# m4tx/idencomp

Measured on NVIDIA B200. Metric: fastq_compress_decompress_GBps, higher is better.
Workload: dtype u32

## Files before the change

idencomp_b200/csrc/idn_device.cuh:

```cuda
#pragma once
#include <cstdint>
#include <cuda_runtime.h>

namespace idn {

constexpr uint32_t kScaleBits = 14;
constexpr uint32_t kAcidSyms = 5, kQSyms = 94;
constexpr uint32_t kSlotMask = (1u << kScaleBits) - 1;
constexpr uint32_t kRansL = 1u << 23;
constexpr int kHist = 8;
constexpr int kQLutBytes = 128;
#ifndef IDN_QROW352
constexpr int kQWindows = 24;
constexpr int kQRowBytes = kQLutBytes + 16 * kQWindows;
#else
constexpr int kQStarts = 104;
constexpr int kQRowBytes = 352;
#endif
constexpr int kQWinBytes = 128 * 16;

struct Magic {
    uint32_t m, s;
};
__host__ __device__ constexpr Magic make_magic(uint32_t d) {
// ... 24 lines not shown
    uint32_t pb;
    uint32_t sbits;
    uint32_t asub, qmul, light;
};

struct SpecBuild {
    SpecDev spec;
    uint32_t total_bits;
    bool ok;
};

__host__ __device__ constexpr uint64_t spec_ipow(uint64_t b, uint32_t n) {
    uint64_t r = 1;
    while (n--) r *= b;
    return r;
}
__host__ __device__ constexpr uint32_t spec_bitlen(uint64_t v) {
    uint32_t n = 0;
    while (v) {
        n++;
        v >>= 1;
    }
    return n;
}

__host__ __device__ constexpr bool make_queue(uint32_t base, uint32_t order, QueueDev& q, uint32_t& bits) {
    q = QueueDev{0, 0, 0, 0, 0, 0, 0, 0, order};
    uint64_t pw = spec_ipow(base, order);
    if (pw > (1ull << 31)) return false;
    bits = spec_bitlen(pw - 1);
    if (order == 0) return true;
    q.vmul = 1;
    uint32_t M = (uint32_t)spec_ipow(base, order - 1);
    q.powmul = M;
    Magic mb = make_magic(base);
    q.mb = mb.m;
    q.shb = mb.s;
    if (order >= 2) {
        q.B = base;
        Magic mm = make_magic(M);
        q.m = mm.m;
        q.sh = mm.s;
        q.MB = (uint32_t)((uint64_t)M * base);
    }
    return true;
}

__host__ __device__ constexpr SpecBuild make_spec(int kind, int ao, int qo, int pb, int qmax) {
    SpecBuild r{SpecDev{QueueDev{0, 0, 0, 0, 0, 0, 0, 0, 0}, QueueDev{0, 0, 0, 0, 0, 0, 0, 0, 0}, 0, 0, 0, 0, 0, 0}, 0, false};
    if (kind != 0 && kind != 1) return r;
    if (ao < 0 || ao > kHist || qo < 0 || qo > kHist || pb < 0 || pb > 16) return r;
    SpecDev& s = r.spec;
    s.pb = (uint32_t)pb;
    s.light = kind == 1;
    uint32_t base_a = 5, base_q = 94;
    s.asub = 0;
    s.qmul = 1u << 20;
    if (s.light) {
        if (qmax < 1 || qmax > 94) return r;
        base_a = 4;
        base_q = (uint32_t)qmax;
        s.asub = 1;
        s.qmul = (uint32_t)qmax * 11156u;
        for (uint32_t q = 0; q < 94; q++)
            if (((q * s.qmul) >> 20) != q * (uint32_t)qmax / 94) return r;
    }
    uint32_t qbits = 0;
    if (!make_queue(base_a, (uint32_t)ao, s.qa, s.abits)) return r;
    if (base_q == 1) {
        s.qq = QueueDev{0, 0, 0, 0, 0, 0, 0, 0, (uint32_t)qo};
        qbits = 0;
    } else if (!make_queue(base_q, (uint32_t)qo, s.qq, qbits)) {
        return r;
    }
    if (s.abits + qbits + s.pb > 31) return r;
    s.sbits = s.abits + qbits;
    r.total_bits = s.abits + qbits + s.pb;
    r.ok = true;
    return r;
}

struct DynSpecs {
    static constexpr bool kStatic = false;
    static constexpr bool kQWin = false;
    __host__ __device__ static constexpr SpecDev sa() { return make_spec(0, 0, 0, 0, 0).spec; }
    __host__ __device__ static constexpr SpecDev sq() { return make_spec(0, 0, 0, 0, 0).spec; }
};
template <int KA, int AOA, int QOA, int PBA, int QMA, int KQ, int AOQ, int QOQ, int PBQ, int QMQ>
struct StaticSpecs {
    static constexpr bool kStatic = true;
#ifdef IDN_QWIN_ALL
    static constexpr bool kQWin = true;
#elif defined(IDN_QWIN_NONE)
    static constexpr bool kQWin = false;
#else
    static constexpr bool kQWin = KQ == 0 && AOQ == 2 && QOQ == 1 && PBQ == 6;
#endif
    __host__ __device__ static constexpr SpecDev sa() { return make_spec(KA, AOA, QOA, PBA, QMA).spec; }
    __host__ __device__ static constexpr SpecDev sq() { return make_spec(KQ, AOQ, QOQ, PBQ, QMQ).spec; }
};

struct ModelDev {
    SpecDev spec;
    uint32_t type, nsym, n_rows;
    const uint16_t* map;
    const uint32_t* hkeys;
    const uint32_t* hvals;
    uint32_t hmask;
    const uint2* enc;
    const uint8_t* dec;
    const uint4* qwin;
    const uint2* adirect;
    const uint2* aenc;
};

__device__ __forceinline__ uint2 ldg_stream8(const uint2* p) {
#ifdef IDN_ACID_NOALLOC
    uint2 v;
    asm volatile("ld.global.nc.L1::no_allocate.v2.u32 {%0, %1}, [%2];" : "=r"(v.x), "=r"(v.y) : "l"(p));
    return v;
#else
    return __ldg(p);
#endif
}

__device__ __forceinline__ uint32_t hash32(uint32_t k) {
    k ^= k >> 16;
    k *= 0x7feb352dU;
    k ^= k >> 15;
    k *= 0x846ca68bU;
    k ^= k >> 16;
    return k;
}

__host__ __device__ constexpr uint32_t spec_table_index(const SpecDev& s, uint32_t spec) {
    return s.pb == 0 ? spec : (((spec & ((1u << s.pb) - 1u)) << s.sbits) | (spec >> s.pb));
}

__device__ __forceinline__ uint32_t ctx_row_hash(const ModelDev& m, uint32_t spec) {
    if (!m.hkeys) return 0;
    uint32_t h = hash32(spec) & m.hmask;
    for (;;) {
        uint32_t k = __ldg(m.hkeys + h);
        if (k == spec) return __ldg(m.hvals + h);
        if (k == 0xffffffffu) return 0;
        h = (h + 1) & m.hmask;
    }
}

template <bool kDense = false, class Gen>
__device__ __forceinline__ uint32_t gen_row(const ModelDev& m, const SpecDev& s, const Gen& g, uint32_t pos_shared, uint32_t pshift) {
    if (kDense || m.map) return __ldg(m.map + g.index(s, pos_shared, pshift));
    return ctx_row_hash(m, g.spec(s, pos_shared, pshift));
}

__device__ __forceinline__ void map_syms(const SpecDev& s, uint32_t a, uint32_t q, bool z, uint32_t& va, uint32_t& vq) {
    va = a - s.asub;
    vq = (q * s.qmul) >> 20;
    const bool kill = z && s.light != 0;
    va = kill ? 0u : va;
    vq = kill ? 0u : vq;
}

__device__ __forceinline__ uint32_t queue_push(const QueueDev& k, uint32_t s, uint32_t v) {
    uint32_t q = __umulhi(s, k.m) >> k.sh;
    return s * k.B - q * k.MB + v * k.vmul;
}
__device__ __forceinline__ uint32_t queue_slide_back(const QueueDev& k, uint32_t s, uint32_t v_old) {
    return (__umulhi(s, k.mb) >> k.shb) + v_old * k.powmul;
}

struct PosFwd {
    uint32_t pos, rem, step, frac, len;
    __device__ __forceinline__ void init(uint32_t length, uint32_t pbmax) {
        len = length ? length : 1;
        uint32_t P = 1u << pbmax;
        step = P / len;
        frac = P - step * len;
        pos = rem = 0;
    }
    __device__ __forceinline__ void init_at(uint32_t length, uint32_t pbmax, uint32_t i) {
        init(length, pbmax);
        const unsigned long long t = (unsigned long long)i << pbmax;
        pos = (uint32_t)(t / len);
        rem = (uint32_t)(t % len);
    }
    __device__ __forceinline__ void advance() {
        pos += step;
        rem += frac;
        if (rem >= len) {
            rem -= len;
            pos++;
        }
    }
};
struct PosBack {
    uint32_t pos, rem, step, frac, len;
    __device__ __forceinline__ void init(uint32_t length, uint32_t pbmax) {
        len = length ? length : 1;
        uint32_t P = 1u << pbmax;
        step = P / len;
        frac = P - step * len;
        pos = P;
        rem = 0;
    }
    __device__ __forceinline__ void init_at(uint32_t length, uint32_t pbmax, uint32_t i) {
        init(length, pbmax);
        const unsigned long long t = (unsigned long long)i << pbmax;
        pos = (uint32_t)(t / len);
        rem = (uint32_t)(t % len);
    }
    __device__ __forceinline__ void retreat() {
        pos -= step;
        if (rem < frac) {
            rem += len;
            pos--;
        }
        rem -= frac;
    }
};

struct GenFwd {
    uint32_t sa, sq;
    __device__ __forceinline__ void init() { sa = sq = 0; }
    __device__ __forceinline__ uint32_t spec(const SpecDev& s, uint32_t pos_shared, uint32_t pshift) const {
        if (s.pb == 0) return (sq << s.abits) | sa;
        return (((sq << s.abits) | sa) << s.pb) | (pos_shared >> pshift);
    }
    __device__ __forceinline__ uint32_t index(const SpecDev& s, uint32_t pos_shared, uint32_t pshift) const {
        if (s.pb == 0) return (sq << s.abits) | sa;
        return ((pos_shared >> pshift) << s.sbits) | ((sq << s.abits) | sa);
    }
    __device__ __forceinline__ void update(const SpecDev& s, uint32_t a, uint32_t q, bool z) {
        uint32_t va, vq;
        map_syms(s, a, q, z, va, vq);
        sa = queue_push(s.qa, sa, va);
        sq = queue_push(s.qq, sq, vq);
    }
};

struct GenBack {
    uint32_t sa, sq;
    uint32_t wa;
    unsigned long long wq;
    uint32_t sha, shq;

    __device__ __forceinline__ void clear(const SpecDev& s) {
        sa = sq = 0;
        wa = 0;
        wq = 0;
        sha = 3 * s.qa.depth;
        shq = 7 * s.qq.depth;
    }
    __device__ __forceinline__ void shift_in(const SpecDev& s, uint32_t a, uint32_t q, bool z) {
        uint32_t va, vq;
        map_syms(s, a, q, z, va, vq);
        wa = (wa >> 3) | (va << (3 * kHist));
        wq = (wq >> 7) | ((unsigned long long)vq << (7 * kHist));
    }
    __device__ __forceinline__ void init_state(const SpecDev& s) {
        sa = sq = 0;
        for (uint32_t k = s.qa.depth; k >= 1; k--) sa = queue_push(s.qa, sa, (wa >> (3 * k)) & 7u);
        for (uint32_t k = s.qq.depth; k >= 1; k--) sq = queue_push(s.qq, sq, (uint32_t)(wq >> (7 * k)) & 127u);
    }
    __device__ __forceinline__ void step_back(const SpecDev& s) {
        sa = queue_slide_back(s.qa, sa, (wa >> sha) & 7u);
        sq = queue_slide_back(s.qq, sq, (uint32_t)(wq >> shq) & 127u);
    }
    __device__ __forceinline__ uint32_t spec(const SpecDev& s, uint32_t pos_shared, uint32_t pshift) const {
        if (s.pb == 0) return (sq << s.abits) | sa;
        return (((sq << s.abits) | sa) << s.pb) | (pos_shared >> pshift);
    }
    __device__ __forceinline__ uint32_t index(const SpecDev& s, uint32_t pos_shared, uint32_t pshift) const {
        if (s.pb == 0) return (sq << s.abits) | sa;
        return ((pos_shared >> pshift) << s.sbits) | ((sq << s.abits) | sa);
    }
};

template <class Out>
__device__ __forceinline__ void rans_put_bf(uint32_t& x, uint2 e, Out& out) {
    const uint32_t freq = (e.y >> 14) & 0x3fffu;
    const uint32_t start = e.y & 0x3fffu;
    const uint32_t x_max = freq << (23 - kScaleBits + 8);
    const bool one = x >= x_max, two = (x >> 8) >= x_max;
    const uint32_t sel = two ? 0x4401u : (one ? 0x4440u : 0x4444u);
    const uint32_t kbits = two ? 16u : (one ? 8u : 0u);
    out.push_bits(__byte_perm(x, 0, sel), kbits);
    x >>= kbits;
    const uint32_t q = freq == 1 ? x : (__umulhi(x, e.x) >> (e.y >> 28));
    x = x + start + q * ((1u << kScaleBits) - freq);
}

__device__ __forceinline__ void rans_put_count(uint32_t& x, uint2 e, uint32_t& bytes) {
    uint32_t freq = (e.y >> 14) & 0x3fffu;
    uint32_t start = e.y & 0x3fffu;
    uint32_t x_max = freq << (23 - kScaleBits + 8);
    const uint32_t k = (x >= x_max ? 1u : 0u) + ((x >> 8) >= x_max ? 1u : 0u);
    bytes += k;
    x >>= 8 * k;
    uint32_t q = freq == 1 ? x : (__umulhi(x, e.x) >> (e.y >> 28));
    x = x + start + q * ((1u << kScaleBits) - freq);
}

__device__ __forceinline__ uint32_t acid_find(uint2 packed, uint32_t slot, uint32_t& start, uint32_t& freq) {
    const uint32_t c1 = packed.x & 0xffffu, c2 = packed.x >> 16, c3 = packed.y & 0xffffu, c4 = packed.y >> 16;
    const bool p1 = slot >= c1, p2 = slot >= c2, p3 = slot >= c3, p4 = slot >= c4;
    start = p4 ? c4 : (p3 ? c3 : (p2 ? c2 : (p1 ? c1 : 0u)));
    const uint32_t next = !p1 ? c1 : (!p2 ? c2 : (!p3 ? c3 : (!p4 ? c4 : (1u << kScaleBits))));
    freq = next - start;
    return p4 ? 4u : (p3 ? 3u : (p2 ? 2u : (p1 ? 1u : 0u)));
}

#ifndef IDN_QROW352
__device__ __forceinline__ uint32_t q_find(const uint8_t* __restrict__ row, uint32_t slot, uint32_t& start,
                                           uint32_t& freq) {
    uint32_t g = __ldg(row + (slot >> 7));
    const uint4* wins = reinterpret_cast<const uint4*>(row + kQLutBytes);
    const uint32_t K = (slot | 0x8000u) * 0x10001u;
    uint4 w = __ldg(wins + g);
    uint32_t flags;
    for (;;) {
        flags = ((K - w.x) & 0x80008000u) | (((K - w.y) & 0x80008000u) >> 1) | (((K - w.z) & 0x80008000u) >> 2) |
                (((K - w.w) & 0x80008000u) >> 3);
#ifndef IDN_ABL_NOADV
        if (!(flags & 0x10000000u)) break;
        g++;
        w = __ldg(wins + g);
#else
        break;
#endif
    }
    const uint32_t j = __popc(flags) - 1;
    const uint32_t p = j >> 1;
    const uint32_t w0 = p == 0 ? w.x : (p == 1 ? w.y : (p == 2 ? w.z : w.w));
    const uint32_t w1 = p == 0 ? w.y : (p == 1 ? w.z : w.w);
    const uint32_t pair = __funnelshift_r(w0, w1, 16 * (j & 1));
    start = pair & 0xffffu;
    freq = (pair >> 16) - start;
    return 4 * g + j;
}
#else
__device__ __forceinline__ uint32_t q_find(const uint8_t* __restrict__ row, uint32_t slot, uint32_t& start,
                                           uint32_t& freq) {
    uint32_t g = __ldg(row + (slot >> 7));
    const uint2* starts = reinterpret_cast<const uint2*>(row + kQLutBytes);
    const uint32_t K = (slot | 0x8000u) * 0x10001u;
    uint2 lo = __ldg(starts + g), hi = __ldg(starts + g + 1);
    uint32_t flags;
    for (;;) {
        flags = ((K - lo.x) & 0x80008000u) | (((K - lo.y) & 0x80008000u) >> 1) | (((K - hi.x) & 0x80008000u) >> 2) |
                (((K - hi.y) & 0x80008000u) >> 3);
        if (!(flags & 0x10000000u)) break;
        g++;
        lo = hi;
        hi = __ldg(starts + g + 1);
    }
    const uint32_t j = __popc(flags) - 1;
    const uint32_t p = j >> 1;
    const uint32_t w0 = p == 0 ? lo.x : (p == 1 ? lo.y : (p == 2 ? hi.x : hi.y));
    const uint32_t w1 = p == 0 ? lo.y : (p == 1 ? hi.x : hi.y);
    const uint32_t pair = __funnelshift_r(w0, w1, 16 * (j & 1));
    start = pair & 0xffffu;
    freq = (pair >> 16) - start;
    return 4 * g + j;
}
#endif

__device__ __forceinline__ uint32_t q_find_win(const uint4* __restrict__ win_row, const uint8_t* __restrict__ row, uint32_t slot,
                                               uint32_t& start, uint32_t& freq) {
    const uint4 w = __ldg(win_row + (slot >> 7));
    const uint32_t K = (slot | 0x8000u) * 0x10001u;
    const uint32_t flags = ((K - w.y) & 0x80008000u) | (((K - w.z) & 0x80008000u) >> 1) | (((K - w.w) & 0x80008000u) >> 2);
    const uint32_t j = __popc(flags);
    if (j == 6) return q_find(row, slot, start, freq);
    const uint32_t i = j + 1;
    const uint32_t p = i >> 1;
    const uint32_t w0 = p == 0 ? w.x : (p == 1 ? w.y : (p == 2 ? w.z : w.w));
    const uint32_t w1 = p == 0 ? w.y : (p == 1 ? w.z : w.w);
    const uint32_t pair = __funnelshift_r(w0, w1, 16 * (i & 1));
    start = pair & 0xffffu;
    freq = (pair >> 16) - start;
    return (w.x & 0xffffu) + j;
}

}
```

idencomp_b200/csrc/idn_kernels.cuh:

```cuda
#pragma once
#include "idn_device.cuh"

namespace idn {

struct BackReader {
    const uint32_t* wp;
    uint32_t word;
    int lane;
    __device__ __forceinline__ void start(const uint8_t* last) {
        const uintptr_t a = reinterpret_cast<uintptr_t>(last);
        wp = reinterpret_cast<const uint32_t*>(a & ~(uintptr_t)3);
        lane = (int)(a & 3) + 4;
        word = 0;
    }
    __device__ __forceinline__ uint32_t get() {
        if (lane >= 4) {
            word = __ldg(wp);
            lane -= 4;
        }
        const uint32_t b = (word >> (8 * lane)) & 0xffu;
        if (--lane < 0) {
            lane = 7;
            wp--;
        }
// ... 1346 lines not shown
            cp_async_wait<0>();
            __syncwarp();
            A = (blk_abs + pos) & ~(uintptr_t)15;
            walk_stage(tiles[cur], A, lo16, hi16, buf_lo, buf_hi, lane);
        }
    }
    cp_async_wait<0>();
    if (lane == 0) {
        blk_reads[b] = n_reads;
        blk_syms[b] = n_syms;
        if (st != 0) {
            int old = atomicCAS(&status[0], 0, st);
            if (old == 0) status[1] = (int32_t)b;
        }
    }
}

constexpr int kWalkFastThreads = 128;
constexpr int kWalkDepth = 6;
constexpr uint32_t kWalkFastMaxBlocks = 512;
constexpr int kWalkFixRounds = 8;
constexpr unsigned long long kWalkNone = ~0ull;

struct WalkHdr {
    uint32_t kind, w1, w2;
};

__device__ __forceinline__ WalkHdr walk_load_hdr(uintptr_t a, uintptr_t buf_lo, uintptr_t buf_hi) {
    const uintptr_t A = a & ~(uintptr_t)7;
    unsigned long long q0 = 0, q1 = 0;
    if (A >= buf_lo && A + 16 <= buf_hi) {
        q0 = __ldg(reinterpret_cast<const unsigned long long*>(A));
        q1 = __ldg(reinterpret_cast<const unsigned long long*>(A + 8));
    } else {
        for (int j = 0; j < 16; j++) {
            const uintptr_t pa = A + j;
            unsigned long long v = (pa >= buf_lo && pa < buf_hi) ? *reinterpret_cast<const uint8_t*>(pa) : 0;
            if (j < 8) q0 |= v << (8 * j);
            else q1 |= v << (8 * (j - 8));
        }
    }
    const uint32_t sh = 8 * (uint32_t)(a & 7);
    const unsigned long long lo = sh ? (q0 >> sh) | (q1 << (64 - sh)) : q0;
    const uint32_t b8 = (uint32_t)(q1 >> sh) & 0xffu;
    WalkHdr h;
    h.kind = (uint32_t)lo & 0xffu;
    h.w1 = __byte_perm((uint32_t)(lo >> 8), 0, 0x0123);
    h.w2 = __byte_perm((uint32_t)(lo >> 40) | (b8 << 24), 0, 0x0123);
    return h;
}

__device__ __forceinline__ unsigned long long walk_slice_size(const WalkHdr& h, unsigned long long room, uint32_t n_models) {
    if (h.kind == 2) return (room < 9 || h.w1 < 8 || h.w1 > room - 9) ? 0 : 9ull + h.w1;
    if (h.kind == 1) return (room < 2 || (h.w1 >> 24) >= n_models || (h.w1 >> 24) >= 255) ? 0 : 2ull;
    if (h.kind == 0) return (room < 6 || h.w1 > room - 6) ? 0 : 6ull + h.w1;
    return 0;
}

__global__ void __launch_bounds__(kWalkFastThreads)
walk_fast_kernel(const uint8_t* __restrict__ blocks, const unsigned long long* __restrict__ block_off,
                 const uint32_t* __restrict__ block_len, uint32_t n_blocks, unsigned long long blocks_bytes,
                 const uint8_t* __restrict__ model_type, uint32_t n_models, const unsigned long long* __restrict__ slot_base,
                 ReadIndexDev ix, unsigned long long* __restrict__ blk_reads, unsigned long long* __restrict__ blk_syms,
                 uint8_t* __restrict__ done, const int32_t* __restrict__ status) {
    __shared__ unsigned long long s_start[kWalkFastThreads];
    __shared__ unsigned long long s_syms[kWalkFastThreads];
    __shared__ uint32_t s_cnt[kWalkFastThreads];
    __shared__ uint32_t s_set[kWalkFastThreads];
    __shared__ int s_fail, s_giveup;
    const uint32_t b = blockIdx.x, t = threadIdx.x;
    if (b >= n_blocks) return;
    if (t == 0) done[b] = 0;
    if (status[0] == 12) return;
    const unsigned long long boff = block_off[b];
    const unsigned long long n = block_len ? block_len[b] : block_off[b + 1] - boff;
    if (boff > blocks_bytes || n > blocks_bytes - boff || n > 0xffffffffull) return;
    const uintptr_t buf_lo = reinterpret_cast<uintptr_t>(blocks), buf_hi = buf_lo + blocks_bytes;
    const uintptr_t blk = buf_lo + boff;
    const uint8_t* bytes = blocks + boff;

    const unsigned long long seg = max(64ull, (n + kWalkFastThreads - 1) / kWalkFastThreads);
    const unsigned long long g0 = min(n, (unsigned long long)t * seg), g1 = min(n, g0 + seg);
    unsigned long long start = kWalkNone;
    if (t == 0) {
        start = 0;
    } else {
        for (unsigned long long p = g0; p < g1; p++) {
            if (__ldg(bytes + p) != 2) continue;
            unsigned long long q = p;
            bool good = true;
            for (int hop = 0; hop < kWalkDepth && q < n; hop++) {
                const unsigned long long sz = walk_slice_size(walk_load_hdr(blk + q, buf_lo, buf_hi), n - q, n_models);
                if (!sz) {
                    good = false;
                    break;
                }
                q += sz;
            }
            if (good) {
                start = p;
                break;
            }
        }
    }
    s_start[t] = start;
    if (t == 0) {
        s_fail = kWalkFastThreads;
        s_giveup = 0;
    }
    __syncthreads();

    unsigned long long next = n, piece_next = kWalkNone;
    uint32_t cnt = 0, set = 0xffffu, need = 0;
    unsigned long long syms = 0, p = 0;
    uint32_t state = 0;
    bool all_ok = false;
    for (int round = 0; round < kWalkFixRounds; round++) {
        start = s_start[t];
        next = n;
        for (uint32_t j = t + 1; j < (uint32_t)kWalkFastThreads; j++)
            if (s_start[j] != kWalkNone) {
                next = s_start[j];
                break;
            }
        if (start == kWalkNone) {
            state = 0;
            cnt = 0;
            syms = 0;
            set = 0xffffu;
            need = 0;
        } else if (next != piece_next) {
            piece_next = next;
            cnt = 0;
            syms = 0;
            set = 0xffffu;
            need = 0;
            state = 0;
            p = start;
            while (p < next) {
                const WalkHdr h = walk_load_hdr(blk + p, buf_lo, buf_hi);
                const unsigned long long sz = walk_slice_size(h, n - p, n_models);
                if (!sz) {
                    state = 2;
                    break;
                }
                if (h.kind == 2) {
                    cnt++;
                    syms += h.w2;
                    need |= ((set & 0xffu) == 0xffu ? 1u : 0u) | ((set >> 8) == 0xffu ? 2u : 0u);
                } else if (h.kind == 1) {
                    const uint32_t idx = h.w1 >> 24;
                    set = model_type[idx] == 0 ? ((set & 0xff00u) | idx) : ((set & 0x00ffu) | (idx << 8));
                }
                p += sz;
            }
            if (state == 0 && p != next) state = 1;
        }
        if (state) atomicMin(&s_fail, (int)t);
        __syncthreads();
        const int f = s_fail;
        __syncthreads();
        if (f == kWalkFastThreads) {
            all_ok = true;
            break;
        }
        if ((int)t == f) {
            if (state == 1 && next != n) {
                for (uint32_t j = t + 1; j < (uint32_t)kWalkFastThreads; j++)
                    if (s_start[j] == next) {
                        s_start[j] = kWalkNone;
                        break;
                    }
            } else {
                s_giveup = 1;
            }
            s_fail = kWalkFastThreads;
        }
        __syncthreads();
        if (s_giveup) return;
    }
    if (!all_ok) return;
    s_cnt[t] = cnt;
    s_syms[t] = syms;
    s_set[t] = set;
    __syncthreads();

    unsigned long long first_read = 0, first_sym = 0;
    uint32_t act = 0xffffu;
    for (uint32_t j = 0; j < t; j++) {
        first_read += s_cnt[j];
        first_sym += s_syms[j];
        const uint32_t sj = s_set[j];
        act = ((sj & 0xffu) != 0xffu ? (sj & 0xffu) : (act & 0xffu)) | ((sj & 0xff00u) != 0xff00u ? (sj & 0xff00u) : (act & 0xff00u));
    }
    const bool active_ok = !(((need & 1u) && (act & 0xffu) == 0xffu) || ((need & 2u) && (act >> 8) == 0xffu));
    if (!__syncthreads_and(active_ok)) return;

    if (start != kWalkNone) {
        const unsigned long long slot0 = slot_base[b] + first_read;
        unsigned long long i = 0, so = first_sym;
        p = start;
        while (p < next) {
            const WalkHdr h = walk_load_hdr(blk + p, buf_lo, buf_hi);
            if (h.kind == 2) {
                ix.pay_off[slot0 + i] = boff + p + 9;
                ix.pay_len[slot0 + i] = h.w1;
                ix.seq_len[slot0 + i] = h.w2;
                ix.sym_off[slot0 + i] = so;
                ix.am[slot0 + i] = (uint8_t)(act & 0xffu);
                ix.qm[slot0 + i] = (uint8_t)(act >> 8);
                so += h.w2;
                i++;
            } else if (h.kind == 1) {
                const uint32_t idx = h.w1 >> 24;
                act = model_type[idx] == 0 ? ((act & 0xff00u) | idx) : ((act & 0x00ffu) | (idx << 8));
            }
            p += walk_slice_size(h, n - p, n_models);
        }
    }
    if (t == kWalkFastThreads - 1) {
        blk_reads[b] = first_read + cnt;
        blk_syms[b] = first_sym + syms;
        done[b] = 1;
    }
}

__global__ void __launch_bounds__(256)
index_check_kernel(const unsigned long long* __restrict__ blk_reads, const unsigned long long* __restrict__ blk_syms,
                   uint32_t n_blocks, uint64_t reads_cap, uint64_t syms_cap, uint32_t* __restrict__ block_first,
                   int32_t* __restrict__ status) {
    uint32_t i = blockIdx.x * blockDim.x + threadIdx.x;
    if (i <= n_blocks && block_first) block_first[i] = (uint32_t)blk_reads[i];
    if (i != 0) return;
    status[3] = 0x7fffffff;
    if (status[0] != 0) return;
    if (blk_reads[n_blocks] > reads_cap || blk_syms[n_blocks] > syms_cap) {
        status[0] = 11;
        status[1] = -1;
        status[2] = (int32_t)(blk_reads[n_blocks] > 0x7fffffffull ? 0x7fffffff : blk_reads[n_blocks]);
    }
}

struct IdentU64 {
    const unsigned long long* v;
    __device__ __forceinline__ unsigned long long operator()(uint64_t i) const { return v[i]; }
};

struct DecodeArgs {
    const ModelDev* models;
    const int32_t* model_ids;
    const uint8_t* payload;
    ReadIndexDev ix;
    const unsigned long long* blk_read_base;
    const unsigned long long* blk_sym_base;
    const unsigned long long* slot_base;
    uint32_t n_blocks;
    uint64_t n_reads;
    const int32_t* status;
    uint8_t* acids_out;
    uint8_t* quals_out;
    long long out_dq;
    unsigned long long* read_off_out;
    uint32_t* read_status;
    uint32_t* err;
    uint32_t* part_crc;
    unsigned long long* part_len;
    const uint32_t* crc_tab;
    const uint32_t* xpow;
};

struct DecStream {
    uint32_t xq, xa;
    unsigned long long w;
    uint32_t bits;
    uint32_t nextw;
    const uint32_t* wp;
    int32_t wleft;
    uint32_t lowest;
    uint32_t st, cur;
    __device__ __forceinline__ uint32_t load_word() {
        uint32_t v = 0;
        if (wleft > 0) v = __ldg(wp);
        wp++;
        wleft--;
        return v;
    }
    __device__ __forceinline__ void begin(const uint8_t* payload, unsigned long long off, uint32_t len) {
        const uintptr_t a = reinterpret_cast<uintptr_t>(payload + off);
        const uint32_t skip = (uint32_t)(a & 3);
        wp = reinterpret_cast<const uint32_t*>(a - skip);
        wleft = len < 8 ? 0 : (int32_t)((skip + len + 3) >> 2);
        const uint32_t w0 = load_word(), w1 = load_word(), w2 = load_word();
        nextw = load_word();
        const uint32_t sh = 8 * skip;
        xq = __funnelshift_r(w0, w1, sh);
        xa = __funnelshift_r(w1, w2, sh);
        w = w2 >> sh;
        bits = 32 - sh;
        lowest = 0xffffffffu;
        st = 0;
        cur = 0;
    }
    __device__ __forceinline__ void refill() {
        if (bits < 32) {
            w |= (unsigned long long)nextw << bits;
            bits += 32;
            nextw = load_word();
        }
    }
    __device__ __forceinline__ void renorm(uint32_t& x) {
        const bool one = x < kRansL, two = x < (1u << 15);
        const uint32_t sel = two ? 0x5401u : (one ? 0x6540u : 0x7654u);
        const uint32_t sh = two ? 16u : (one ? 8u : 0u);
        x = __byte_perm((uint32_t)w, x, sel);
        w >>= sh;
        bits -= sh;
    }
    __device__ __forceinline__ void renorm_all() {
        renorm(xq);
        renorm(xa);
        lowest = min(lowest, min(xq, xa));
    }
    __device__ __forceinline__ void finish(const uint8_t* payload, unsigned long long off, uint32_t len) {
        const uint32_t skip = (uint32_t)(reinterpret_cast<uintptr_t>(payload + off) & 3);
        const int32_t nw = len < 8 ? 0 : (int32_t)((skip + len + 3) >> 2);
        const int32_t in_window = nw - wleft - 1;
        const int32_t used = 4 * in_window - (int32_t)skip - (int32_t)(bits >> 3);
        cur = (uint32_t)used;
        st = (len < 8 || used > (int32_t)len || lowest < kRansL) ? 1u : 0u;
    }
    __device__ __forceinline__ bool clean_end(uint32_t len) const { return xq == kRansL && xa == kRansL && cur == len; }
};

struct SymWriter {
    uint8_t* pa;
    long long dq;
#ifndef IDN_NO_SYM16
    uint32_t an_lo, an_hi;
    uint32_t q0, q1, q2, q3;
    uint32_t nw;
#endif
    __device__ __forceinline__ void init(uint8_t* a, long long dq_) {
        pa = a;
        dq = dq_;
#ifndef IDN_NO_SYM16
        an_lo = an_hi = q0 = q1 = q2 = q3 = 0;
        nw = (dq_ & 15) == 0 ? 0x80000000u : 0u;
#endif
    }
    __device__ __forceinline__ bool aligned() const {
        return ((reinterpret_cast<uintptr_t>(pa) | (uintptr_t)dq) & 3) == 0;
    }
#ifndef IDN_NO_SYM16
    static __device__ __forceinline__ uint32_t pack4(uint32_t w) {
        const uint32_t t = w | (w >> 4);
        return __byte_perm(t, 0, 0x4420);
    }
    static __device__ __forceinline__ uint32_t unpack4(uint32_t n16) {
        const uint32_t t = __byte_perm(n16, 0, 0x4140);
        return (t | (t << 4)) & 0x0f0f0f0fu;
    }
    __device__ __forceinline__ void flush() {
        const uint32_t k = nw & 3u;
        uint32_t* wa = reinterpret_cast<uint32_t*>(pa);
        uint32_t* wq = reinterpret_cast<uint32_t*>(pa + dq);
        if (k == 3) {
            wa[-3] = unpack4(an_lo >> 16);
            wq[-3] = q1;
        }
        if (k >= 2) {
            wa[-2] = unpack4(an_hi & 0xffffu);
            wq[-2] = q2;
        }
        if (k >= 1) {
            wa[-1] = unpack4(an_hi >> 16);
            wq[-1] = q3;
        }
        nw &= 0x80000000u;
    }
#else
    __device__ __forceinline__ void flush() {}
#endif
    __device__ __forceinline__ void put(uint32_t a, uint32_t q) {
#ifndef IDN_NO_SYM16
        if (nw & 3u) flush();
#endif
        pa[0] = (uint8_t)a;
        pa[dq] = (uint8_t)q;
        pa++;
    }
    __device__ __forceinline__ void put4(uint32_t wa, uint32_t wq) {
#ifdef IDN_ABL_NOSTORE
        if (wa != 0xdeadbeefu) { pa += 4; return; }
#endif
#ifndef IDN_NO_SYM16
        if ((nw & 3u) || (nw && (reinterpret_cast<uintptr_t>(pa) & 15) == 0)) {
            an_lo = __funnelshift_r(an_lo, an_hi, 16);
            an_hi = __byte_perm(an_hi, pack4(wa), 0x5432);
            q0 = q1; q1 = q2; q2 = q3; q3 = wq;
            pa += 4;
            nw++;
            if ((nw & 7u) == 4) {
                *reinterpret_cast<uint4*>(pa - 16) = make_uint4(unpack4(an_lo & 0xffffu), unpack4(an_lo >> 16),
                                                                unpack4(an_hi & 0xffffu), unpack4(an_hi >> 16));
                *reinterpret_cast<uint4*>(pa + dq - 16) = make_uint4(q0, q1, q2, q3);
                nw &= 0x80000000u;
            }
            return;
        }
#endif
        *reinterpret_cast<uint32_t*>(pa) = wa;
        *reinterpret_cast<uint32_t*>(pa + dq) = wq;
        pa += 4;
    }
};

struct DecCrc {
    const uint32_t* tab;
    uint32_t ca, cq;
};

template <class P>
__device__ __forceinline__ void decode_read_body(const ModelDev& ma, const ModelDev& mq, uint32_t len, uint32_t p0, uint32_t p1,
                                                 const uint8_t* __restrict__ hist, DecStream& D, SymWriter& O, DecCrc& C) {
    constexpr SpecDev ksa = P::sa(), ksq = P::sq();
    const SpecDev& sa = P::kStatic ? ksa : ma.spec;
    const SpecDev& sq = P::kStatic ? ksq : mq.spec;
    GenFwd ga, gq;
    ga.init();
    gq.init();
    const uint32_t pbmax = sa.pb > sq.pb ? sa.pb : sq.pb;
    const uint32_t psa = pbmax - sa.pb, psq = pbmax - sq.pb;
    PosFwd pf;
    pf.init_at(len, pbmax, p0);
    if (p0) {
#pragma unroll 1
        for (int k = 0; k < kHist; k++) {
            uint32_t ha = __ldg(hist + k), hq = __ldg(hist + kHist + k);
            ha = ha > 4 ? 0 : ha;
            hq = hq > 93 ? 0 : hq;
            const bool hz = ha * hq == 0;
            ga.update(sa, ha, hq, hz);
            gq.update(sq, ha, hq, hz);
        }
    }
    auto step = [&](uint32_t& va, uint32_t& vq) {
        D.refill();
        uint2 pk;
        if (P::kStatic || ma.adirect) pk = ldg_stream8(ma.adirect + ga.index(sa, pf.pos, psa));
        else pk = __ldg(reinterpret_cast<const uint2*>(ma.dec) + gen_row(ma, sa, ga, pf.pos, psa));
#if defined(IDN_ABL_ROW1)
        const uint32_t row_q = 1;
#elif defined(IDN_ABL_NOQMAP)
        const uint32_t row_q = (gq.spec(sq, pf.pos, psq) * 2654435761u >> 22) + 1;
#else
        const uint32_t row_q = gen_row<P::kStatic>(mq, sq, gq, pf.pos, psq);
#endif
        const uint32_t slot_q = D.xq & kSlotMask, slot_a = D.xa & kSlotMask;
        uint32_t start, freq;
#ifndef IDN_NO_QWIN
        if (P::kQWin) vq = q_find_win(mq.qwin + row_q * (uint32_t)(kQWinBytes / 16), mq.dec + row_q * (uint32_t)kQRowBytes, slot_q, start, freq);
        else
#endif
            vq = q_find(mq.dec + row_q * (uint32_t)kQRowBytes, slot_q, start, freq);
        D.xq = freq * (D.xq >> kScaleBits) + slot_q - start;
        va = acid_find(pk, slot_a, start, freq);
        D.xa = freq * (D.xa >> kScaleBits) + slot_a - start;
        D.renorm_all();
        if (C.tab) {
            C.ca = C.tab[(C.ca ^ va) & 0xffu] ^ (C.ca >> 8);
            C.cq = C.tab[(C.cq ^ vq) & 0xffu] ^ (C.cq >> 8);
        }
        const bool z = va * vq == 0;
        ga.update(sa, va, vq, z);
        gq.update(sq, va, vq, z);
        pf.advance();
    };
    uint32_t i = p0, va, vq;
#pragma unroll 1
    for (; i < p1 && !O.aligned(); i++) {
        step(va, vq);
        O.put(va, vq);
    }
#pragma unroll 1
    for (; i + 4 <= p1; i += 4) {
        uint32_t wa, wq;
        step(wa, wq);
        step(va, vq);
        wa = __byte_perm(wa, va, 0x3240);
        wq = __byte_perm(wq, vq, 0x3240);
        step(va, vq);
        wa = __byte_perm(wa, va, 0x3410);
        wq = __byte_perm(wq, vq, 0x3410);
        step(va, vq);
        wa = __byte_perm(wa, va, 0x4210);
        wq = __byte_perm(wq, vq, 0x4210);
        O.put4(wa, wq);
    }
#pragma unroll 1
    for (; i < p1; i++) {
        step(va, vq);
        O.put(va, vq);
    }
}

__device__ __forceinline__ bool decode_locate(const DecodeArgs& A, uint64_t r, unsigned long long& slot, unsigned long long& sym_base) {
    const unsigned long long R = A.blk_read_base[A.n_blocks];
    if (r >= R) return false;
    uint32_t lo = 0, hi = A.n_blocks;
    while (hi - lo > 1) {
        uint32_t mid = (lo + hi) >> 1;
        if (__ldg(A.blk_read_base + mid) <= r) lo = mid; else hi = mid;
    }
    slot = A.slot_base[lo] + (r - A.blk_read_base[lo]);
    sym_base = A.blk_sym_base[lo];
    return true;
}

template <bool kUniform, class P>
__device__ __forceinline__ void decode_one(const DecodeArgs& A, const ModelDev& MA, const ModelDev& MQ, uint64_t r, const uint32_t* s_tab,
                                           const uint32_t* s_xpow) {
    DecCrc C{A.part_crc ? s_tab : nullptr, 0xffffffffu, 0xffffffffu};
    unsigned long long slot = r, sym_base = 0;
    if (A.blk_read_base) {
        if (!decode_locate(A, r, slot, sym_base)) return;
        const unsigned long long R = A.blk_read_base[A.n_blocks];
        if (r == R - 1 && A.read_off_out) A.read_off_out[R] = A.blk_sym_base[A.n_blocks];
    } else if (r >= A.n_reads) {
        return;
    }
    const ModelDev& ma = kUniform ? MA : A.models[A.model_ids[A.ix.am[slot]]];
    const ModelDev& mq = kUniform ? MQ : A.models[A.model_ids[A.ix.qm[slot]]];
    const uint32_t len = A.ix.seq_len[slot];
    const unsigned long long ooff = sym_base + A.ix.sym_off[slot];
    if (A.read_off_out) A.read_off_out[r] = ooff;
    DecStream D;
    D.begin(A.payload, A.ix.pay_off[slot], A.ix.pay_len[slot]);
    SymWriter O;
    O.init(A.acids_out + ooff, A.out_dq);
    decode_read_body<P>(ma, mq, len, 0, len, nullptr, D, O, C);
    O.flush();
    const uint32_t plen = A.ix.pay_len[slot];
    D.finish(A.payload, A.ix.pay_off[slot], plen);
    uint32_t st = D.st;
    if (!(st & 1) && !D.clean_end(plen)) st |= 2;
    if (A.read_status) A.read_status[r] = st;
    if (st) atomicOr(A.err, 1u);
    if (A.part_crc) {
        const CrcPair p = crc_concat(CrcPair{~C.ca, len}, CrcPair{~C.cq, len}, s_xpow);
        A.part_crc[r] = len ? p.crc : 0u;
        A.part_len[r] = 2ull * len;
    }
}

template <bool kUniform, class P>
__global__ void __launch_bounds__(128, kUniform ? IDN_DEC_MINB : 1)
decode_kernel(DecodeArgs A, const ModelDev MA, const ModelDev MQ) {
    __shared__ uint32_t s_tab[256];
    __shared__ uint32_t s_xpow[64];
    uint64_t r = (uint64_t)blockIdx.x * blockDim.x + threadIdx.x;
    if (A.status && A.status[0] != 0) return;
    if (A.part_crc) {
        for (int k = threadIdx.x; k < 256; k += blockDim.x) s_tab[k] = A.crc_tab[k];
        for (int k = threadIdx.x; k < 64; k += blockDim.x) s_xpow[k] = A.xpow[k];
        __syncthreads();
    }
    decode_one<kUniform, P>(A, MA, MQ, r, s_tab, s_xpow);
}

template <class P>
__global__ void __launch_bounds__(128, IDN_DEC_MINB)
decode_list_kernel(DecodeArgs A, const ModelDev MA, const ModelDev MQ, ReadList L) {
    __shared__ uint32_t s_tab[256];
    __shared__ uint32_t s_xpow[64];
    if (A.status && A.status[0] != 0) return;
    if (A.part_crc) {
        for (int k = threadIdx.x; k < 256; k += blockDim.x) s_tab[k] = A.crc_tab[k];
        for (int k = threadIdx.x; k < 64; k += blockDim.x) s_xpow[k] = A.xpow[k];
        __syncthreads();
    }
    const uint32_t n = *L.count;
    const uint32_t* __restrict__ list = L.list + *L.base;
    for (uint64_t i = (uint64_t)blockIdx.x * blockDim.x + threadIdx.x; i < n; i += (uint64_t)gridDim.x * blockDim.x)
        decode_one<true, P>(A, MA, MQ, list[i], s_tab, s_xpow);
}

struct DecodePairKey {
    DecodeArgs A;
    uint32_t n_models;
    __device__ __forceinline__ uint32_t operator()(uint64_t r) const {
        if (A.status && A.status[0] != 0) return 0xffffffffu;
        unsigned long long slot, sym_base;
        if (!decode_locate(A, r, slot, sym_base)) return 0xffffffffu;
        return (uint32_t)A.ix.am[slot] * n_models + A.ix.qm[slot];
    }
};

__global__ void finish_decode_kernel(const int32_t* __restrict__ status, const uint32_t* __restrict__ err,
                                     const unsigned long long* __restrict__ n_reads_total,
                                     const unsigned long long* __restrict__ n_syms_total,
                                     unsigned long long* __restrict__ read_off_out, int32_t* __restrict__ status_dev) {
    if (threadIdx.x != 0 || blockIdx.x != 0) return;
    int32_t code = status[0];
    uint64_t R = *n_reads_total;
    int32_t blk = status[1];
    if (code == 0 && (*err & 1u)) code = 3;
    if (code == 6) blk = status[3];
    status_dev[0] = code;
    status_dev[1] = blk;
    status_dev[2] = code == 11 ? status[2] : (int32_t)(R > 0x7fffffffull ? 0x7fffffff : R);
    status_dev[3] = (int32_t)(*n_syms_total & 0x7fffffffull);
    if (code == 0 && R == 0 && read_off_out) read_off_out[0] = 0;
}

__device__ __forceinline__ unsigned long long splitmix64(unsigned long long& s) {
    unsigned long long z = (s += 0x9E3779B97F4A7C15ull);
    z = (z ^ (z >> 30)) * 0xBF58476D1CE4E5B9ull;
    z = (z ^ (z >> 27)) * 0x94D049BB133111EBull;
    return z ^ (z >> 31);
}

__global__ void __launch_bounds__(128)
synth_kernel(const ModelDev* __restrict__ models, int32_t ia, int32_t iq, const unsigned long long* __restrict__ read_off,
             uint64_t n_reads, uint64_t first_read_index, unsigned long long seed, uint32_t n_ppm,
             uint8_t* __restrict__ acids, uint8_t* __restrict__ quals) {
    uint64_t r = (uint64_t)blockIdx.x * blockDim.x + threadIdx.x;
    if (r >= n_reads) return;
    const ModelDev& ma = models[ia];
    const ModelDev& mq = models[iq];
    unsigned long long off = read_off[r];
    uint32_t len = (uint32_t)(read_off[r + 1] - off);
    unsigned long long s = seed ^ ((first_read_index + r + 1) * 0xD1B54A32D192ED03ull);
    const SpecDev sa = ma.spec, sq = mq.spec;
    GenFwd ga, gq;
    ga.init();
    gq.init();
    const uint32_t pbmax = sa.pb > sq.pb ? sa.pb : sq.pb;
    const uint32_t psa = pbmax - sa.pb, psq = pbmax - sq.pb;
    PosFwd pf;
    pf.init(len, pbmax);
    FwdWriter oa, oq;
    oa.init(acids + off);
    oq.init(quals + off);
    uint32_t prev_q = 0;
    for (uint32_t i = 0; i < len; i++) {
        unsigned long long u = splitmix64(s);
        uint32_t slot_a = (uint32_t)u & kSlotMask, slot_q = (uint32_t)(u >> 14) & kSlotMask;
        uint32_t start, freq;
        uint32_t row_a = gen_row(ma, sa, ga, pf.pos, psa);
        uint32_t row_q = gen_row(mq, sq, gq, pf.pos, psq);
        uint2 pk = __ldg(reinterpret_cast<const uint2*>(ma.dec) + row_a);
        uint32_t a = acid_find(pk, slot_a, start, freq);
        uint32_t q = q_find(mq.dec + row_q * (uint32_t)kQRowBytes, slot_q, start, freq);
        if (row_a == 0) a = 1 + (slot_a & 3u);
        if (row_q == 0 && i > 0) q = prev_q;
        if ((uint32_t)((u >> 32) % 1000000u) < n_ppm) {
            a = 0;
            q = 2;
        }
        prev_q = q;
        oa.push(a);
        oq.push(q);
        const bool z = a * q == 0;
        ga.update(sa, a, q, z);
        gq.update(sq, a, q, z);
        pf.advance();
    }
    oa.finish();
    oq.finish();
}

}
```

Before: 283.7.

## Branchless symbol lookup, predicated refill, and templated word-wise CRC in decoder

After: 293.3, median of 6. 1.03x the previous value.

```diff
diff --git a/idencomp_b200/csrc/idn_device.cuh b/idencomp_b200/csrc/idn_device.cuh
--- a/idencomp_b200/csrc/idn_device.cuh
+++ b/idencomp_b200/csrc/idn_device.cuh
@@ -350,13 +350,23 @@
     x = x + start + q * ((1u << kScaleBits) - freq);
 }
 
+__device__ __forceinline__ uint32_t start_pair(uint4 w, uint32_t j) {
+    const bool b1 = j & 2u, b2 = j & 4u;
+    const uint32_t w0 = b2 ? (b1 ? w.w : w.z) : (b1 ? w.y : w.x);
+    const uint32_t w1 = b2 ? w.w : (b1 ? w.z : w.y);
+    return __funnelshift_r(w0, w1, 16 * (j & 1));
+}
+
 __device__ __forceinline__ uint32_t acid_find(uint2 packed, uint32_t slot, uint32_t& start, uint32_t& freq) {
-    const uint32_t c1 = packed.x & 0xffffu, c2 = packed.x >> 16, c3 = packed.y & 0xffffu, c4 = packed.y >> 16;
-    const bool p1 = slot >= c1, p2 = slot >= c2, p3 = slot >= c3, p4 = slot >= c4;
-    start = p4 ? c4 : (p3 ? c3 : (p2 ? c2 : (p1 ? c1 : 0u)));
-    const uint32_t next = !p1 ? c1 : (!p2 ? c2 : (!p3 ? c3 : (!p4 ? c4 : (1u << kScaleBits))));
-    freq = next - start;
-    return p4 ? 4u : (p3 ? 3u : (p2 ? 2u : (p1 ? 1u : 0u)));
+    const uint32_t K = (slot | 0x8000u) * 0x10001u;
+    const uint32_t flags = ((K - packed.x) & 0x80008000u) | (((K - packed.y) & 0x80008000u) >> 1);
+    const uint32_t s = __popc(flags);
+    const uint32_t lo = s == 0 ? 0u : (s < 3 ? packed.x : packed.y);
+    const uint32_t hi = s < 2 ? packed.x : (s < 4 ? packed.y : (1u << kScaleBits));
+    const uint32_t pair = __funnelshift_r(lo, hi, 16 * (~s & 1u));
+    start = pair & 0xffffu;
+    freq = (pair >> 16) - start;
+    return s;
 }
 
 #ifndef IDN_QROW352
@@ -365,24 +375,23 @@
     uint32_t g = __ldg(row + (slot >> 7));
     const uint4* wins = reinterpret_cast<const uint4*>(row + kQLutBytes);
     const uint32_t K = (slot | 0x8000u) * 0x10001u;
+    auto win_flags = [K](uint4 v) {
+        return ((K - v.x) & 0x80008000u) | (((K - v.y) & 0x80008000u) >> 1) | (((K - v.z) & 0x80008000u) >> 2) |
+               (((K - v.w) & 0x80008000u) >> 3);
+    };
     uint4 w = __ldg(wins + g);
-    uint32_t flags;
-    for (;;) {
-        flags = ((K - w.x) & 0x80008000u) | (((K - w.y) & 0x80008000u) >> 1) | (((K - w.z) & 0x80008000u) >> 2) |
-                (((K - w.w) & 0x80008000u) >> 3);
+    uint32_t flags = win_flags(w);
 #ifndef IDN_ABL_NOADV
-        if (!(flags & 0x10000000u)) break;
-        g++;
-        w = __ldg(wins + g);
-#else
-        break;
+    if (__builtin_expect((flags & 0x10000000u) != 0, 0)) {
+        do {
+            g++;
+            w = __ldg(wins + g);
+            flags = win_flags(w);
+        } while (flags & 0x10000000u);
+    }
 #endif
-    }
     const uint32_t j = __popc(flags) - 1;
-    const uint32_t p = j >> 1;
-    const uint32_t w0 = p == 0 ? w.x : (p == 1 ? w.y : (p == 2 ? w.z : w.w));
-    const uint32_t w1 = p == 0 ? w.y : (p == 1 ? w.z : w.w);
-    const uint32_t pair = __funnelshift_r(w0, w1, 16 * (j & 1));
+    const uint32_t pair = start_pair(w, j);
     start = pair & 0xffffu;
     freq = (pair >> 16) - start;
     return 4 * g + j;
@@ -404,10 +413,7 @@
         hi = __ldg(starts + g + 1);
     }
     const uint32_t j = __popc(flags) - 1;
-    const uint32_t p = j >> 1;
-    const uint32_t w0 = p == 0 ? lo.x : (p == 1 ? lo.y : (p == 2 ? hi.x : hi.y));
-    const uint32_t w1 = p == 0 ? lo.y : (p == 1 ? hi.x : hi.y);
-    const uint32_t pair = __funnelshift_r(w0, w1, 16 * (j & 1));
+    const uint32_t pair = start_pair(make_uint4(lo.x, lo.y, hi.x, hi.y), j);
     start = pair & 0xffffu;
     freq = (pair >> 16) - start;
     return 4 * g + j;
@@ -421,11 +427,7 @@
     const uint32_t flags = ((K - w.y) & 0x80008000u) | (((K - w.z) & 0x80008000u) >> 1) | (((K - w.w) & 0x80008000u) >> 2);
     const uint32_t j = __popc(flags);
     if (j == 6) return q_find(row, slot, start, freq);
-    const uint32_t i = j + 1;
-    const uint32_t p = i >> 1;
-    const uint32_t w0 = p == 0 ? w.x : (p == 1 ? w.y : (p == 2 ? w.z : w.w));
-    const uint32_t w1 = p == 0 ? w.y : (p == 1 ? w.z : w.w);
-    const uint32_t pair = __funnelshift_r(w0, w1, 16 * (i & 1));
+    const uint32_t pair = start_pair(w, j + 1);
     start = pair & 0xffffu;
     freq = (pair >> 16) - start;
     return (w.x & 0xffffu) + j;
diff --git a/idencomp_b200/csrc/idn_kernels.cuh b/idencomp_b200/csrc/idn_kernels.cuh
--- a/idencomp_b200/csrc/idn_kernels.cuh
+++ b/idencomp_b200/csrc/idn_kernels.cuh
@@ -1672,11 +1672,14 @@
         cur = 0;
     }
     __device__ __forceinline__ void refill() {
-        if (bits < 32) {
-            w |= (unsigned long long)nextw << bits;
-            bits += 32;
-            nextw = load_word();
-        }
+        const bool need = bits < 32;
+        uint32_t v = 0;
+        if (need && wleft > 0) v = __ldg(wp);
+        w |= (unsigned long long)(need ? nextw : 0u) << bits;
+        bits += need ? 32u : 0u;
+        nextw = need ? v : nextw;
+        wp += need ? 1 : 0;
+        wleft -= need ? 1 : 0;
     }
     __device__ __forceinline__ void renorm(uint32_t& x) {
         const bool one = x < kRansL, two = x < (1u << 15);
@@ -1790,9 +1793,19 @@
     uint32_t ca, cq;
 };
 
-template <class P>
-__device__ __forceinline__ void decode_read_body(const ModelDev& ma, const ModelDev& mq, uint32_t len, uint32_t p0, uint32_t p1,
-                                                 const uint8_t* __restrict__ hist, DecStream& D, SymWriter& O, DecCrc& C) {
+__device__ __forceinline__ uint32_t crc_byte(uint32_t c, uint32_t b, const uint32_t* __restrict__ tab) {
+    return tab[(c ^ b) & 0xffu] ^ (c >> 8);
+}
+__device__ __forceinline__ uint32_t crc_word(uint32_t c, uint32_t w, const uint32_t* __restrict__ tab) {
+    c ^= w;
+#pragma unroll
+    for (int k = 0; k < 4; k++) c = tab[c & 0xffu] ^ (c >> 8);
+    return c;
+}
+
+template <class P, bool kCrc>
+__device__ __forceinline__ void decode_read_positions(const ModelDev& ma, const ModelDev& mq, uint32_t len, uint32_t p0, uint32_t p1,
+                                                      const uint8_t* __restrict__ hist, DecStream& D, SymWriter& O, DecCrc& C) {
     constexpr SpecDev ksa = P::sa(), ksq = P::sq();
     const SpecDev& sa = P::kStatic ? ksa : ma.spec;
     const SpecDev& sq = P::kStatic ? ksq : mq.spec;
@@ -1837,10 +1850,6 @@
         va = acid_find(pk, slot_a, start, freq);
         D.xa = freq * (D.xa >> kScaleBits) + slot_a - start;
         D.renorm_all();
-        if (C.tab) {
-            C.ca = C.tab[(C.ca ^ va) & 0xffu] ^ (C.ca >> 8);
-            C.cq = C.tab[(C.cq ^ vq) & 0xffu] ^ (C.cq >> 8);
-        }
         const bool z = va * vq == 0;
         ga.update(sa, va, vq, z);
         gq.update(sq, va, vq, z);
@@ -1850,6 +1859,10 @@
 #pragma unroll 1
     for (; i < p1 && !O.aligned(); i++) {
         step(va, vq);
+        if (kCrc) {
+            C.ca = crc_byte(C.ca, va, C.tab);
+            C.cq = crc_byte(C.cq, vq, C.tab);
+        }
         O.put(va, vq);
     }
 #pragma unroll 1
@@ -1865,13 +1878,28 @@
         step(va, vq);
         wa = __byte_perm(wa, va, 0x4210);
         wq = __byte_perm(wq, vq, 0x4210);
+        if (kCrc) {
+            C.ca = crc_word(C.ca, wa, C.tab);
+            C.cq = crc_word(C.cq, wq, C.tab);
+        }
         O.put4(wa, wq);
     }
 #pragma unroll 1
     for (; i < p1; i++) {
         step(va, vq);
+        if (kCrc) {
+            C.ca = crc_byte(C.ca, va, C.tab);
+            C.cq = crc_byte(C.cq, vq, C.tab);
+        }
         O.put(va, vq);
     }
+}
+
+template <class P>
+__device__ __forceinline__ void decode_read_body(const ModelDev& ma, const ModelDev& mq, uint32_t len, uint32_t p0, uint32_t p1,
+                                                 const uint8_t* __restrict__ hist, DecStream& D, SymWriter& O, DecCrc& C) {
+    if (C.tab) decode_read_positions<P, true>(ma, mq, len, p0, p1, hist, D, O, C);
+    else decode_read_positions<P, false>(ma, mq, len, p0, p1, hist, D, O, C);
 }
 
 __device__ __forceinline__ bool decode_locate(const DecodeArgs& A, uint64_t r, unsigned long long& slot, unsigned long long& sym_base) {
```
